# main--/rust-lz-fear

Hardware: AMD Instinct MI355X
Metric: GiB/s compress + decompress, 4 MiB independent blocks, 1/2/4/8 MI355X (higher is better)
Workload: dtype u8

## Files before the change

rust-lz-fear_amd/csrc/lz4_decompress_batch_phase.inc:

```
            LZF_STAGE_NEEDS(jv, DecodeJob); LZF_STAGE_NEEDS(rg.kRing, uint32_t); LZF_STAGE_NEEDS(sb.kCB, uint32_t); LZF_STAGE_NEEDS(lane, uint32_t);
            LZF_STAGE_NEEDS(o, uint32_t); LZF_STAGE_NEEDS(safe, uint32_t); LZF_STAGE_NEEDS(status, int); LZF_STAGE_NEEDS(cstart, uint32_t); LZF_STAGE_NEEDS(Tc, uint32_t);
            static_assert(kSpanMax + kNearHist == rg.kRing, "a batch's span and the intact history share the ring");
#if defined(LZF_FED_DECODE)
            LZF_STAGE_NEEDS(expect, uint32_t); LZF_STAGE_NEEDS(fed_carry, uint32_t); LZF_STAGE_NEEDS(bail, bool); LZF_STAGE_NEEDS(toks[0], uint16_t);
#elif !defined(LZF_TOKEN_AT)
#error "lz4_decompress_batch_phase.inc: define LZF_TOKEN_AT(i) (or LZF_FED_DECODE) around the include"
#endif
            uint32_t tidx = 0;
            if (LZF_DBG_SKIP & 1) { tidx = Tc; o += Tc; }
#if defined(LZF_FED_DECODE)
            if (LZF_DBG_SKIP & 1) expect = jv.len;
#endif
            while (tidx < Tc && status == LZF_OK) {
#if defined(LZF_FED_DECODE)
                if (lzf_fedw_carry(Tc, tidx, cstart + kRound, jv.len, fed_carry)) break;
#endif
                PHASE(0);
#if defined(LZF_DBG_ROUNDS) && defined(LZF_DBG_ROUNDS_HERE)
                ++dbg_batches;
#endif
#if defined(LZF_FED_DECODE) && defined(LZF_DBG_FED_COUNT)
                ++dbg_fed[0];
#endif
                const uint32_t ob0 = o;
                const uint32_t nb_try = Tc - tidx < kWave ? Tc - tidx : kWave;
#if defined(LZF_FED_DECODE)
                const unsigned long long act0 = lanes_below(nb_try);
#else
                const bool act0 = lane < nb_try;
#endif
                uint32_t L = 0, M = 0, src = 0;
                bool has = false;
#if defined(LZF_FED_DECODE)
                uint32_t next;
                const uint32_t pos = toks[tidx + lane_sel(act0, lane, 0u)];
                const uint32_t tp = cstart + pos;
                uint32_t w;
                asm volatile("ds_read_b32 %0, %1\n\ts_waitcnt lgkmcnt(0)" : "=v"(w) : "v"(sb.lds + pos) : "memory");
                const uint32_t l0 = (w >> 4) & 15u, b1 = (w >> 8) & 255u, m0 = w & 15u;
                const bool lx = l0 == 15u;
                const uint32_t lext = lx ? b1 : 0u;
                L = l0 + lext;
                src = tp + (lx ? 2u : 1u);
                const uint32_t q = src + L;
                has = q + 2u <= jv.len;
                const bool mx = has && m0 == 15u;
                uint32_t rq = q - cstart;
                const bool fit4 = rq + 4u <= sb.kCB;
                const uint32_t ow = lds_ld32(sb.lds + (fit4 ? rq : 0u));
                uint32_t off = ow & 0xFFFFu;
                const uint32_t mext = mx ? (fit4 ? (ow >> 16) & 255u : 255u) : 0u;
                M = has ? m0 + 4u + mext : 0u;
                uint32_t need = has ? q + (mx ? 3u : 2u) : q;
                next = has ? need : jv.len;
                const bool general = (lext > mext ? lext : mext) == 255u;
                {
                    if (general) {
                        uint32_t p = tp + 1u, b = 0;
                        bool bad = false;
                        L = l0; M = 0; has = false; next = jv.len;
                        if (lx) {
                            do { if (p >= jv.len) { bad = true; break; } b = sb.rdb(p); ++p; L += b; if (L > kMaxPosB) L = kMaxPosB; } while (b == 255u);
                        }
                        src = p;
                        if (!bad && jv.len - p < L) bad = true;
                        p += L;
                        if (!bad && jv.len - p >= 2u) {
                            has = true; p += 2u; M = m0;
                            if (m0 == 15u) {
                                do { if (p >= jv.len) { bad = true; break; } b = sb.rdb(p); ++p; M += b; if (M > kMaxPosB) M = kMaxPosB; } while (b == 255u);
                            }
                            M += 4u; next = p;
                        }
                        need = bad ? 0xFFFFFFFFu : 0u;
                        rq = sb.kCB;
                    }
                }
                if ((__builtin_amdgcn_uicmp(need, jv.len, 34 ) | __builtin_amdgcn_uicmp(tp, wave_prev(next, expect), 33 )) & act0) { bail = true; break; }
#else
#ifdef LZF_TOKEN_WORD
                bool decode = act0;
                if (act0) {
                    const uint32_t tw = LZF_TOKEN_WORD(tidx + lane);
                    const uint32_t lc = (tw >> 16) & 255u, mc = tw >> 24;
                    if (lc != 255u && mc != 255u) {
                        decode = false;
                        L = lc; src = cstart + (tw & 0xFFFFu) + (lc >= 15u ? 2u : 1u);
                        if (mc != 254u) { has = true; M = mc + 4u; }
                    }
                }
                if (decode) {
#else
                if (act0) {
#endif
                    const uint32_t tp = cstart + LZF_TOKEN_AT(tidx + lane);
                    const uint32_t w = sb.rd4(tp);
                    const uint32_t tok = w & 255u;
                    uint32_t q = tp + 1u;
                    L = tok >> 4;
                    if (L == 15u) {
                        uint32_t b = (w >> 8) & 255u; ++q;
                        L += b;
                        while (b == 255u) { b = sb.rdb(q); ++q; L += b; if (L > kMaxPosB) L = kMaxPosB; }
                    }
                    src = q; q += L;
                    if (jv.len - q >= 2u) {
                        has = true; q += 2u;
                        M = tok & 15u;
                        if (M == 15u) { for (;;) { const uint32_t b = sb.rdb(q); ++q; M += b; if (M > kMaxPosB) M = kMaxPosB; if (b != 255u) break; } }
                        M += 4u;
                    }
                }
#endif
                uint32_t tot = L + M; if (tot > kTotClamp || tot < L) tot = kTotClamp;
#if defined(LZF_FED_DECODE)
                const uint32_t tot0 = lane_sel(act0, tot, 0u);
                const uint32_t incl = wave_scan_add(tot0);
                const uint32_t lo = ob0 + (incl - tot0);
                const uint32_t mo = lo + L;
                const uint32_t nb = first_lane_min(__builtin_amdgcn_uicmp(incl, kSpanMax, 34 ), nb_try);
#else
                const uint32_t incl = wave_scan_add(act0 ? tot : 0u);
                const uint32_t lo = ob0 + (incl - (act0 ? tot : 0u));
                const uint32_t mo = lo + L;
                const uint32_t c = first_lane(__ballot(act0 && incl > kSpanMax));
                const uint32_t nb = c < nb_try ? c : nb_try;
#endif

                if (nb == 0u) {
#if defined(LZF_FED_DECODE)
                    expect = __builtin_amdgcn_readlane(next, 0);
#endif
                    const uint32_t s_L = __builtin_amdgcn_readlane(L, 0);
                    const uint32_t s_M = __builtin_amdgcn_readlane(M, 0);
                    const uint32_t s_src = __builtin_amdgcn_readlane(src, 0);
                    const bool s_has = __builtin_amdgcn_readlane((uint32_t)has, 0) != 0u;
                    if (jv.cap - o < s_L) { status = LZF_OUT_CAPACITY; break; }
                    if (s_has && (uint64_t)o + s_L + s_M > jv.limit) { status = LZF_MEMORY_LIMIT_EXCEEDED; break; }
                    const uint32_t o_before = o;
                    wave_copy(jv.out + o, jv.in + s_src, s_L, lane);
                    o += s_L;
                    if (s_has) {
                        const uint32_t offset = (uint32_t)jv.in[s_src + s_L] | ((uint32_t)jv.in[s_src + s_L + 1u] << 8);
                        uint32_t mlen = s_M;
                        if (offset == 0u) { status = LZF_ZERO_DEDUP_OFFSET; break; }
                        bool done = false;
                        if (offset > o) {
                            const uint32_t need = offset - o;
                            if (need > jv.plen) { status = LZF_INVALID_DEDUP_OFFSET; break; }
                            const uint32_t nn = need < mlen ? need : mlen;
                            if (jv.cap - o < nn) { status = LZF_OUT_CAPACITY; break; }
                            wave_copy(jv.out + o, jv.prefix + (jv.plen - need), nn, lane);
                            o += nn; mlen -= nn;
                            done = mlen == 0u;
                        }
                        if (!done) {
                            if (jv.cap - o < mlen) { status = LZF_OUT_CAPACITY; break; }
                            const uint32_t src0 = o - offset;
                            const uint32_t span = mlen < offset ? mlen : offset;
                            if (src0 + span > safe) { wave_store_fence(); safe = o; }
                            cgu8* hist = jv.out + src0;
                            gu8* dst = jv.out + o;
                            if (mlen <= offset) {
                                wave_copy(dst, hist, mlen, lane);
                            } else if (offset == 1u) {
                                const uint32_t b = hist[0];
                                const uint32_t b4 = b * 0x01010101u;
                                const u32x4 v = {b4, b4, b4, b4};
                                const uint32_t bulk = mlen & ~15u;
                                for (uint32_t i = lane * 16u; i < bulk; i += kWave * 16u) st16(dst + i, v);
                                if (lane < mlen - bulk) dst[bulk + lane] = (uint8_t)b;
                            } else {
                                uint32_t r = lane % offset;
                                const uint32_t adv = kWave % offset;
                                for (uint32_t i = lane; i < mlen; i += kWave) {
                                    dst[i] = hist[r];
                                    r += adv; if (r >= offset) r -= offset;
                                }
                            }
                            o += mlen;
                        }
                    }
                    wave_store_fence(); safe = o;
                    rg.fill((o - o_before > rg.kRing) ? o - rg.kRing : o_before, o);
                    tidx += 1u;
                    continue;
                }

#if defined(LZF_FED_DECODE)
                expect = __builtin_amdgcn_readlane(next, nb - 1u);
                const unsigned long long act_m = lanes_below(nb);
                L = lane_sel(act_m, L, 0u); M = lane_sel(act_m, M, 0u);
                has = M != 0u;
                const unsigned long long has_m = __builtin_amdgcn_uicmp(M, 0u, 33 );
                const bool act = lane < nb;
                if (__builtin_amdgcn_uicmp(rq, sb.kCB - 4u, 34 ) & has_m) {
                    asm volatile("");
                    if (has && rq > sb.kCB - 4u) {
                        if (!sb.kStage) off = ld2(jv.in + src + L);
                        else if (src + L - cstart + 2u <= sb.kCB) off = lds_ld16(sb.lds + (src + L - cstart));
                        else off = sb.rdb(src + L) | (sb.rdb(src + L + 1u) << 8);
                    }
                }
#else
                const bool act = lane < nb;
                has = has && act;
                if (!act) { L = 0; M = 0; }
                uint32_t off = 0;
                if (has) {
                    if (!sb.kStage) off = ld2(jv.in + src + L);
                    else if (src + L - cstart + 2u <= sb.kCB) off = lds_ld16(sb.lds + (src + L - cstart));
                    else off = sb.rdb(src + L) | (sb.rdb(src + L + 1u) << 8);
                }
#endif
#if defined(LZF_FED_DECODE)
                static_assert(kSpanMax < kTotClamp && (uint64_t)kMaxPosB * 2u < (1ull << 32), "the bounds argument above");
                const uint32_t lim32 = jv.limit > 0xFFFFFFFFull ? 0xFFFFFFFFu : (uint32_t)jv.limit;
                const uint32_t fit = jv.cap < lim32 ? jv.cap : lim32;
                const uint32_t E = ob0 + __builtin_amdgcn_readlane(incl, nb - 1u);
                const unsigned long long flagged = (__builtin_amdgcn_uicmp(off - 1u, mo + jv.plen, 35 ) & has_m) | __builtin_amdgcn_uicmp(E, fit, 34 );
                if (flagged) {
#endif
                int code = LZF_OK;
                if (act) {
                    if (lo > jv.cap || jv.cap - lo < L) code = LZF_OUT_CAPACITY;
                    else if (has && (uint64_t)mo + M > jv.limit) code = LZF_MEMORY_LIMIT_EXCEEDED;
                    else if (has && off == 0u) code = LZF_ZERO_DEDUP_OFFSET;
                    else if (has && off > mo && off - mo > jv.plen) code = LZF_INVALID_DEDUP_OFFSET;
                    else if (has && jv.cap - mo < M) code = LZF_OUT_CAPACITY;
                }
                const uint32_t e = first_lane(__ballot(code != LZF_OK));
                if (e < 64u) { status = __builtin_amdgcn_readlane(code, e); break; }
#if defined(LZF_FED_DECODE)
                }
#endif
                PHASE(1);

                const uint32_t near_lo = ob0 > kNearHist ? ob0 - kNearHist : 0u;
                const uint32_t span = M < off ? M : off;
                const bool from_prefix = has && off > mo;
                const uint32_t s0 = mo - off;
                const bool is_near = has && !from_prefix && s0 >= near_lo;
                const bool is_far = has && !from_prefix && s0 + span <= near_lo;
                const bool is_slow = has && !is_near && !is_far;
                const uint32_t mi = RIDX(mo);
                const bool mwrap = mi + M > rg.kRing;
                {
                    uint32_t need = 0;
                    if (is_far) need = s0 + M;
                    if (is_slow && !from_prefix) need = near_lo;
                    if (is_slow && from_prefix && M > off - mo) need = near_lo;
                    if (need > ob0) need = ob0;
                    if (__ballot(need > safe)) { wave_store_fence(); safe = ob0; }
                }
                const bool far_own = !(LZF_DBG_SKIP & 4) && is_far && M <= kFarShort && !mwrap;
                uint64_t fv0 = 0, fv1 = 0, fv2 = 0, fv3 = 0;
#ifndef LZF_FAR_LATE
                if (far_own) {
                    cgu8* g = jv.out + s0;
                    if (M >= 8u) {
                        fv0 = ld8(g); fv3 = ld8(g + M - 8u);
                        if (M > 16u) { fv1 = ld8(g + 8u); fv2 = ld8(g + M - 16u); }
                    } else {
                        fv0 = ld4(g); fv3 = ld4(g + M - 4u);
                    }
                }
#endif
                if (!(LZF_DBG_SKIP & 8) && __ballot(L > 0u)) {
                    const uint32_t n1 = L < kShort ? L : kShort;
                    const uint32_t ri = RIDX(lo);
                    if (n1 > 0u) {
                        if (ri + n1 > rg.kRing) {
                            for (uint32_t t = 0; t < n1; ++t) rg.ring[RIDX(lo + t)] = (uint8_t)sb.rdb(src + t);
                        } else if (sb.kStage && src - cstart + n1 <= sb.kCB) {
                            put_small_lds(rg.lds + ri, sb.lds + (src - cstart), n1);
                        } else {
                            put_small_glb(rg.lds + ri, jv.in + src, n1);
                        }
                    }
                    for (unsigned long long m = __ballot(L > kShort); m; m &= m - 1ull) {
                        const uint32_t j = (uint32_t)__builtin_ctzll(m);
                        const uint32_t jl = __builtin_amdgcn_readlane(L, j);
                        const uint32_t js = __builtin_amdgcn_readlane(src, j);
                        const uint32_t jo = __builtin_amdgcn_readlane(lo, j);
                        for (uint32_t i = kShort + lane; i < jl; i += 4u * kWave) {
                            const uint32_t i1 = i + kWave, i2 = i + 2u * kWave, i3 = i + 3u * kWave;
                            const uint8_t b0 = jv.in[js + i];
                            const uint8_t b1 = i1 < jl ? jv.in[js + i1] : (uint8_t)0;
                            const uint8_t b2 = i2 < jl ? jv.in[js + i2] : (uint8_t)0;
                            const uint8_t b3 = i3 < jl ? jv.in[js + i3] : (uint8_t)0;
                            rg.ring[RIDX(jo + i)] = b0;
                            if (i1 < jl) rg.ring[RIDX(jo + i1)] = b1;
                            if (i2 < jl) rg.ring[RIDX(jo + i2)] = b2;
                            if (i3 < jl) rg.ring[RIDX(jo + i3)] = b3;
                        }
                    }
                }
                PHASE(2);

#ifdef LZF_FAR_LATE
                if (far_own) {
                    cgu8* g = jv.out + s0;
                    if (M >= 8u) {
                        fv0 = ld8(g); fv3 = ld8(g + M - 8u);
                        if (M > 16u) { fv1 = ld8(g + 8u); fv2 = ld8(g + M - 16u); }
                    } else {
                        fv0 = ld4(g); fv3 = ld4(g + M - 4u);
                    }
                }
#endif
                if (far_own) {
                    const uint32_t dsta = rg.lds + mi;
                    if (M >= 8u) {
                        lds_st64(dsta, fv0);
                        if (M > 16u) { lds_st64(dsta + 8u, fv1); lds_st64(dsta + M - 16u, fv2); }
                        lds_st64(dsta + M - 8u, fv3);
                    } else {
                        lds_st32(dsta, (uint32_t)fv0); lds_st32(dsta + M - 4u, (uint32_t)fv3);
                    }
                }
                if (!(LZF_DBG_SKIP & 4) && __ballot(is_far && !far_own)) {
                    if (is_far && M <= kShort && mwrap) { for (uint32_t t = 0; t < M; ++t) rg.ring[RIDX(mo + t)] = jv.out[s0 + t]; }
                    if (is_far && M > kFarShort && M <= kShort && !mwrap) put_small_glb(rg.lds + mi, jv.out + s0, M);
                    for (unsigned long long m = __ballot(is_far && M > kShort); m; m &= m - 1ull) {
                        const uint32_t j = (uint32_t)__builtin_ctzll(m);
                        const uint32_t jm = __builtin_amdgcn_readlane(M, j);
                        const uint32_t js = __builtin_amdgcn_readlane(s0, j);
                        const uint32_t jo = __builtin_amdgcn_readlane(mo, j);
                        for (uint32_t i = lane; i < jm; i += 4u * kWave) {
                            const uint32_t i1 = i + kWave, i2 = i + 2u * kWave, i3 = i + 3u * kWave;
                            const uint8_t b0 = jv.out[js + i];
                            const uint8_t b1 = i1 < jm ? jv.out[js + i1] : (uint8_t)0;
                            const uint8_t b2 = i2 < jm ? jv.out[js + i2] : (uint8_t)0;
                            const uint8_t b3 = i3 < jm ? jv.out[js + i3] : (uint8_t)0;
                            rg.ring[RIDX(jo + i)] = b0;
                            if (i1 < jm) rg.ring[RIDX(jo + i1)] = b1;
                            if (i2 < jm) rg.ring[RIDX(jo + i2)] = b2;
                            if (i3 < jm) rg.ring[RIDX(jo + i3)] = b3;
                        }
                    }
                }
                PHASE(3);
                unsigned long long unresolved = __ballot(is_near || is_slow);
                const unsigned long long slow_mask = __ballot(is_slow);
                {
                    const uint32_t si = RIDX(s0);
                    const bool solo_ok = is_near && M <= off && M <= kShort && !mwrap && !(si + M > rg.kRing);
                    const unsigned long long solo_mask = __ballot(solo_ok);
                    uint32_t src_end = solo_ok ? s0 + span : 0xFFFFFFFFu;
                    if (LZF_DBG_SKIP & 2) unresolved = 0;
                    while (unresolved) {
#if defined(LZF_DBG_ROUNDS) && defined(LZF_DBG_ROUNDS_HERE)
                        ++dbg_rounds;
#endif
#if defined(LZF_FED_DECODE) && defined(LZF_DBG_FED_COUNT)
                        ++dbg_fed[3];
#endif
                        const uint32_t f = (uint32_t)__builtin_ctzll(unresolved);
                        const unsigned long long bit = 1ull << f;
                        if (solo_mask & bit) {
                            const uint32_t H = __builtin_amdgcn_readlane(mo, f);
                            const bool mine = src_end <= H;
                            if (mine) { put_match_lds(rg.lds + mi, rg.lds + si, M); src_end = 0xFFFFFFFFu; }
#if defined(LZF_DBG_ROUNDS) && defined(LZF_DBG_ROUNDS_HERE) && LZF_DBG_ROUNDS >= 3
                            { const uint32_t nl = (uint32_t)__builtin_popcountll(__ballot(mine));
                              dbg_lane_stat += LZF_DBG_ROUNDS == 3 ? nl : LZF_DBG_ROUNDS == 4 ? 1u : LZF_DBG_ROUNDS == 5 ? (nl == 1u) : LZF_DBG_ROUNDS == 6 ? (nl >= 2u && nl <= 4u)
                                             : LZF_DBG_ROUNDS == 7 ? (nl >= 5u && nl <= 16u) : (nl >= 17u); }
#endif
                            unresolved &= ~__ballot(mine);
                            continue;
                        }
                        unresolved &= ~bit;
                        if (slow_mask & bit) {
                            if (lane == f) {
                                for (uint32_t t = 0; t < M; ++t) {
                                    uint8_t v;
                                    if (off > mo + t) v = jv.prefix[jv.plen - (off - mo) + t];
                                    else {
                                        const uint32_t s = mo + t - off;
                                        v = s < near_lo ? jv.out[s] : rg.ring[RIDX(s)];
                                    }
                                    rg.ring[RIDX(mo + t)] = v;
                                }
                            }
                            continue;
                        }
                        const uint32_t jm = __builtin_amdgcn_readlane(M, f);
                        const uint32_t js = __builtin_amdgcn_readlane(s0, f);
                        const uint32_t jo = __builtin_amdgcn_readlane(mo, f);
                        const uint32_t joff = __builtin_amdgcn_readlane(off, f);
                        if (jm <= joff) {
                            for (uint32_t i = lane; i < jm; i += 4u * kWave) {
                                const uint32_t i1 = i + kWave, i2 = i + 2u * kWave, i3 = i + 3u * kWave;
                                const uint8_t b0 = rg.ring[RIDX(js + i)];
                                const uint8_t b1 = i1 < jm ? rg.ring[RIDX(js + i1)] : (uint8_t)0;
                                const uint8_t b2 = i2 < jm ? rg.ring[RIDX(js + i2)] : (uint8_t)0;
                                const uint8_t b3 = i3 < jm ? rg.ring[RIDX(js + i3)] : (uint8_t)0;
                                rg.ring[RIDX(jo + i)] = b0;
                                if (i1 < jm) rg.ring[RIDX(jo + i1)] = b1;
                                if (i2 < jm) rg.ring[RIDX(jo + i2)] = b2;
                                if (i3 < jm) rg.ring[RIDX(jo + i3)] = b3;
                            }
#if defined(LZF_FED_DECODE)
                        } else if ((LZF_DBG_SKIP & 64) && joff <= 8u && ((0x116u >> joff) & 1u)) {
#endif
                        } else {
#if defined(LZF_FED_DECODE) && !defined(LZF_FED_NO_PERIODIC)
                            uint32_t rr = lane & (joff - 1u), adv = kWave & (joff - 1u);
                            if ((joff & (joff - 1u)) != 0u) {
                                asm volatile("");
                                rr = lane % joff; adv = kWave % joff;
                            }
#if defined(LZF_DBG_FED_COUNT)
                            dbg_fed[4] += (joff & (joff - 1u)) == 0u ? 1u : 0u;
#endif
#else
                            uint32_t rr = lane % joff;
                            const uint32_t adv = kWave % joff;
#endif
                            for (uint32_t i = lane; i < jm; i += kWave) {
                                rg.ring[RIDX(jo + i)] = rg.ring[RIDX(js + rr)];
                                rr += adv; if (rr >= joff) rr -= joff;
                            }
                        }
                    }
                }
                PHASE(4);
                o = ob0 + __builtin_amdgcn_readlane(incl, (nb - 1u) & 63u);
                if (!(LZF_DBG_SKIP & 16)) rg.flush(ob0, o);
                tidx += nb;
                PHASE(5);
            }
```

rust-lz-fear_amd/csrc/lz4_decompress_fed.hip:

```cpp
#include "lzf_device.h"
#include "kernels.h"
#include "lzf_copy_helpers.h"
#include "lzf_phase_timers.h"
#include "lzf_fed_window.h"
#include "lzf_dispatch.h"

namespace lzf {

__device__ __forceinline__ uint32_t xcc_id() {
    uint32_t v; asm volatile("s_getreg_b32 %0, hwreg(HW_REG_XCC_ID)" : "=s"(v)); return v & 15u;
}

template <int RING, int W, int TOKCAP>
__global__ LZF_FED_BOUNDS void lzf_decompress_fed_kernel(fed_args a) {
    constexpr uint32_t kSpanMax = RING / 3;
    constexpr uint32_t kNearHist = RING - kSpanMax;
    constexpr uint32_t kRound = 32u * (uint32_t)W;
    constexpr uint32_t kCB = kRound + 128u;
    static_assert(W >= 1 && W <= 64 && kRound == (uint32_t)kFedwRound, "a window is one bit-map word per lane (whose owner is worked out per word: lzf_fed_window.h)");
    static_assert(TOKCAP >= (int)(kRound / 3u + 1u), "a round's tokens (at least three bytes each) fit the list");
    static_assert(kCB % 16 == 0, "the round is staged in 16-byte pieces");
    __shared__ __attribute__((aligned(16))) uint8_t ring[RING];
    __shared__ __attribute__((aligned(16))) uint8_t cbuf[kCB];
    __shared__ __attribute__((aligned(16))) uint16_t toks[TOKCAP];
    static_assert(RING != 4096 || W != 32 || TOKCAP != 352 || lzf_dispatch::lds_alloc(sizeof ring + sizeof cbuf + sizeof toks) == lzf_dispatch::kFedLdsAlloc, "lzf_dispatch.h: the residency the census falls back on");

    const uint32_t lane = threadIdx.x;
    if (a.census) {
        if (lane == 0u) {
            __hip_atomic_fetch_or(&a.census[2], 1u << (xcc_id() & 31u), __ATOMIC_RELAXED, __HIP_MEMORY_SCOPE_AGENT);
            __hip_atomic_fetch_add(&a.census[0], 1u, __ATOMIC_RELAXED, __HIP_MEMORY_SCOPE_AGENT);
            const unsigned long long t0 = wall_clock64();
            while (wall_clock64() - t0 < 30000ull) __builtin_amdgcn_s_sleep(16);
            const uint32_t seen = __hip_atomic_load(&a.census[0], __ATOMIC_RELAXED, __HIP_MEMORY_SCOPE_AGENT);
            __hip_atomic_fetch_min(&a.census[1], seen, __ATOMIC_RELAXED, __HIP_MEMORY_SCOPE_AGENT);
        }
        return;
    }
    const uint32_t n = a.n_jobs, pieces = a.pieces;
    const uint32_t xcc = xcc_id() & 31u;
    if (pieces > 1u && !((a.xcc_mask >> xcc) & 1u)) return;
    const uint32_t ng = pieces > 1u ? (uint32_t)__popc(a.xcc_mask) : 1u, g = pieces > 1u ? (uint32_t)__popc(a.xcc_mask & ((1u << xcc) - 1u)) : 0u;
    const uint32_t n_g = lzf_fedw_group_jobs(n, g, ng);
#ifdef LZF_ANALYSIS
    const uint32_t n_tickets = n_g * (a.stop_piece && a.stop_piece < pieces ? a.stop_piece : pieces);
#else
    const uint32_t n_tickets = n_g * pieces;
#endif
    for (;;) {
    uint32_t tk = 0;
    if (lane == 0u) tk = __hip_atomic_fetch_add(a.ticket + g * kFedTicketStride, 1u, __ATOMIC_RELAXED, __HIP_MEMORY_SCOPE_AGENT);
    tk = __builtin_amdgcn_readfirstlane(tk);
    if (tk >= n_tickets) break;
    const uint32_t piece = lzf_fedw_ticket_piece(tk, n_g), k = lzf_fedw_ticket_rank(tk, piece, n_g, g, ng);
    const uint32_t jid = a.perm ? a.perm[k] : k;
    const seg_job sj = a.st[jid];
    if (!sj.eligible || sj.failed || sj.done) continue;
    LZF_GLOBAL fed_state* const fs = (LZF_GLOBAL fed_state*)a.state + jid;
    const lzf_decompress_job job = a.jobs[jid];
    const long long t_start = clock64();
#ifdef LZF_DBG_TIMELINE
    const unsigned long long t_wall0 = wall_clock64();
#endif

    int status = LZF_OK;
    bool bailed = false, parked = false;
    uint32_t o = 0;
    PhaseTimers ph;
#ifdef LZF_DBG_FED_COUNT
    uint32_t dbg_fed[5] = {0u, 0u, 0u, 0u, 0u};
#endif
    if (LZF_DECODE_JOB_OUT_OF_CONTRACT(job)) continue;
    {
        const DecodeJob jv = LZF_DECODE_JOB_VIEW(job);
        const OutRing<RING> rg{ring, jv.out, jv.rb, lane, lds_addr(ring)};
        const uint32_t cbuf_a = lds_addr(cbuf);
        const LZF_GLOBAL uint32_t* const fed_bits = (const LZF_GLOBAL uint32_t*)a.bits + (size_t)jid * a.maxch * kSegChunkWords;
        uint32_t expect = 0;
        uint32_t cstart = 0;
        o = (uint32_t)job.out_existing_len;
        const uint32_t piece_end = lzf_fedw_piece_end(jv.len, pieces, piece);
        if (piece > 0u) {
            uint32_t f = 0;
            for (uint32_t spin = 0; spin < (1u << 22); ++spin) {
                f = __hip_atomic_load(&fs->flag, __ATOMIC_RELAXED, __HIP_MEMORY_SCOPE_AGENT);
                if (f >= piece) break;
                __builtin_amdgcn_s_sleep(32);
            }
            f = __builtin_amdgcn_readfirstlane(f);
            if (f != piece) continue;
            __builtin_amdgcn_fence(__ATOMIC_ACQUIRE, "agent");
            expect = fs->expect; o = fs->o;
        }
        uint32_t safe = o;
        if (o > 0) rg.fill(o > (uint32_t)RING ? o - RING : 0u, o);
        ph.start();
#if defined(LZF_FED_FIXED_ROUNDS)
        constexpr int kFixed = 1;
        const uint32_t fed_carry = 0u;
#elif defined(LZF_ANALYSIS)
        constexpr int kFixed = 0;
        const uint32_t fed_carry = a.carry < kWave ? a.carry : kWave - 1u;
#else
        constexpr int kFixed = 0;
        constexpr uint32_t fed_carry = kFedwCarry;
#endif
        bool fed_walk = false;
        while (expect < jv.len && status == LZF_OK) {
            if (expect >= piece_end) { parked = true; break; }
            const uint32_t expect_in = expect;
            cstart = lzf_fedw_start(expect, kFixed);
            __syncthreads();
#ifdef LZF_DBG_FED_COUNT
            ++dbg_fed[fed_walk ? 2 : 1];
#endif
#include "lz4_decompress_feed_phase.inc"
            if (Tc) {
#define LZF_FED_DECODE
#ifdef LZF_FED_FAR_LATE
#define LZF_FAR_LATE
#endif
#include "lz4_decompress_batch_phase.inc"
#undef LZF_FAR_LATE
#undef LZF_FED_DECODE
            }
            if (bail) {
                if (fed_walk) { bailed = true; break; }
                fed_walk = true; continue;
            }
            fed_walk = false;
            if (expect == expect_in && status == LZF_OK) { bailed = true; break; }
        }
        if (parked && status == LZF_OK && !bailed) {
            if (lane == 0u) { fs->expect = expect; fs->o = o; }
            __builtin_amdgcn_fence(__ATOMIC_RELEASE, "workgroup");
            asm volatile("s_waitcnt vmcnt(0)" ::: "memory");
            if (lane == 0u) __hip_atomic_store(&fs->flag, piece + 1u, __ATOMIC_RELAXED, __HIP_MEMORY_SCOPE_AGENT);
            continue;
        }
    }
    if (pieces > 1u && lane == 0u) __hip_atomic_store(&fs->flag, kFedEnded, __ATOMIC_RELAXED, __HIP_MEMORY_SCOPE_AGENT);
    if (bailed || status != LZF_OK) continue;
    if (lane == 0) {
        a.results[jid].out_len = o;
        a.results[jid].status = LZF_OK;
#ifdef LZF_DBG_FED_COUNT
        a.results[jid].reserved = dbg_fed[LZF_DBG_FED_COUNT];
#elif defined(LZF_DBG_PHASE_SEL)
        ph.report(a.results[jid]);
#elif defined(LZF_DBG_TIMELINE)
        a.results[jid].reserved = (uint32_t)(((t_wall0 >> 8) & 0xFFFFull) << 16) | (uint32_t)((wall_clock64() >> 8) & 0xFFFFull);
#else
        a.results[jid].reserved = (uint32_t)((clock64() - t_start) >> 10);
#endif
        a.st[jid].done = 1u;
    }
    }
}

__global__ __launch_bounds__(256) void lzf_fed_reset_kernel(fed_args a) {
    const uint32_t k = blockIdx.x * blockDim.x + threadIdx.x;
    if (k < 32u) a.ticket[k * kFedTicketStride] = 0u;
    if (k < a.n_jobs) a.state[k].flag = 0u;
}

#define LZF_INSTF(NAME, RG, W_, T) template __global__ void lzf_decompress_fed_kernel<RG, W_, T>(fed_args);
LZF_FED_VARIANTS(LZF_INSTF)
#undef LZF_INSTF

}
```

rust-lz-fear_amd/csrc/lzf_out_ring.h:

```cpp
#ifndef LZF_OUT_RING_H
#define LZF_OUT_RING_H

#include <stdint.h>
#if defined(__HIPCC__) || defined(__CUDACC__)
#define LZF_RING_HD __host__ __device__
#else
#define LZF_RING_HD
#endif
struct lzf_ring_parts { uint32_t head, vec, tail; };

LZF_RING_HD constexpr lzf_ring_parts lzf_ring_split(uint32_t a, uint32_t b, uint32_t rb) {
    uint32_t nh = (16u - ((a + rb) & 15u)) & 15u;
    if (nh > b - a) nh = b - a;
    a += nh;
    const uint32_t nv = (b - a) >> 4;
    a += nv << 4;
    return lzf_ring_parts{nh, nv, b - a};
}

#if defined(__HIPCC__)
#include "lzf_device.h"

namespace lzf {
namespace {

#define RIDX(x) (((x) + rg.rb) & (rg.kRing - 1u))
template <int RING>
struct OutRing {
    static_assert(RING >= 16 && (RING & (RING - 1)) == 0, "ring index = address mod RING");
    static constexpr uint32_t kRing = RING;
    uint8_t* ring;
    gu8* out;
    uint32_t rb;
    uint32_t lane;
    uint32_t lds;
    __device__ __forceinline__ uint32_t idx(uint32_t x) const { const OutRing& rg = *this; return RIDX(x); }
    __device__ __forceinline__ uint8_t& at(uint32_t x) const { return ring[idx(x)]; }
    template <bool FLUSH>
    __device__ __forceinline__ void move(uint32_t a, uint32_t b) const {
        const lzf_ring_parts s = lzf_ring_split(a, b, rb);
        if (lane < s.head) { if (FLUSH) out[a + lane] = at(a + lane); else at(a + lane) = out[a + lane]; }
        a += s.head;
        for (uint32_t c = lane; c < s.vec; c += kWave) {
            LZF_GLOBAL u32x4* const g = reinterpret_cast<LZF_GLOBAL u32x4*>(out + a + 16u * c);
            u32x4* const r = reinterpret_cast<u32x4*>(&at(a + 16u * c));
            if (FLUSH) *g = *r; else *r = *g;
        }
        a += s.vec << 4;
        if (lane < s.tail) { if (FLUSH) out[a + lane] = at(a + lane); else at(a + lane) = out[a + lane]; }
    }
    __device__ __forceinline__ void fill(uint32_t a, uint32_t b) const { move<false>(a, b); }
    __device__ __forceinline__ void flush(uint32_t a, uint32_t b) const { move<true>(a, b); }
};

}
}
#endif
#endif
```

Measured before the change: 545.3.

## Defer ring flush of each batch into the next batch's match phase

Result: faster. 552.2 (median of 6 runs) (+1.3%).

```diff
diff --git a/rust-lz-fear_amd/csrc/lz4_decompress_batch_phase.inc b/rust-lz-fear_amd/csrc/lz4_decompress_batch_phase.inc
--- a/rust-lz-fear_amd/csrc/lz4_decompress_batch_phase.inc
+++ b/rust-lz-fear_amd/csrc/lz4_decompress_batch_phase.inc
@@ -2,14 +2,15 @@
             LZF_STAGE_NEEDS(o, uint32_t); LZF_STAGE_NEEDS(safe, uint32_t); LZF_STAGE_NEEDS(status, int); LZF_STAGE_NEEDS(cstart, uint32_t); LZF_STAGE_NEEDS(Tc, uint32_t);
             static_assert(kSpanMax + kNearHist == rg.kRing, "a batch's span and the intact history share the ring");
 #if defined(LZF_FED_DECODE)
-            LZF_STAGE_NEEDS(expect, uint32_t); LZF_STAGE_NEEDS(fed_carry, uint32_t); LZF_STAGE_NEEDS(bail, bool); LZF_STAGE_NEEDS(toks[0], uint16_t);
+            LZF_STAGE_NEEDS(expect, uint32_t); LZF_STAGE_NEEDS(fed_carry, uint32_t); LZF_STAGE_NEEDS(bail, bool); LZF_STAGE_NEEDS(toks[0], uint16_t); LZF_STAGE_NEEDS(pend, uint32_t);
+            static_assert(kSpanMax + 16u <= kNearHist, "the batch before and the ragged end before it lie inside the history this batch keeps intact, above every far source");
 #elif !defined(LZF_TOKEN_AT)
 #error "lz4_decompress_batch_phase.inc: define LZF_TOKEN_AT(i) (or LZF_FED_DECODE) around the include"
 #endif
             uint32_t tidx = 0;
             if (LZF_DBG_SKIP & 1) { tidx = Tc; o += Tc; }
 #if defined(LZF_FED_DECODE)
-            if (LZF_DBG_SKIP & 1) expect = jv.len;
+            if (LZF_DBG_SKIP & 1) { expect = jv.len; pend = o; }
 #endif
             while (tidx < Tc && status == LZF_OK) {
 #if defined(LZF_FED_DECODE)
@@ -130,6 +131,8 @@
                 if (nb == 0u) {
 #if defined(LZF_FED_DECODE)
                     expect = __builtin_amdgcn_readlane(next, 0);
+                    if (!(LZF_DBG_SKIP & 16)) rg.flush(pend, o);
+                    pend = 0xFFFFFFFFu;
 #endif
                     const uint32_t s_L = __builtin_amdgcn_readlane(L, 0);
                     const uint32_t s_M = __builtin_amdgcn_readlane(M, 0);
@@ -183,6 +186,9 @@
                     }
                     wave_store_fence(); safe = o;
                     rg.fill((o - o_before > rg.kRing) ? o - rg.kRing : o_before, o);
+#if defined(LZF_FED_DECODE)
+                    pend = o;
+#endif
                     tidx += 1u;
                     continue;
                 }
@@ -251,7 +257,16 @@
                     if (is_slow && !from_prefix) need = near_lo;
                     if (is_slow && from_prefix && M > off - mo) need = near_lo;
                     if (need > ob0) need = ob0;
+#if defined(LZF_FED_DECODE)
+                    if (__ballot(need > safe)) {
+#if defined(LZF_DBG_FED_COUNT)
+                        ++dbg_fed[5];
+#endif
+                        wave_store_fence(); safe = pend;
+                    }
+#else
                     if (__ballot(need > safe)) { wave_store_fence(); safe = ob0; }
+#endif
                 }
                 const bool far_own = !(LZF_DBG_SKIP & 4) && is_far && M <= kFarShort && !mwrap;
                 uint64_t fv0 = 0, fv1 = 0, fv2 = 0, fv3 = 0;
@@ -341,6 +356,12 @@
                     }
                 }
                 PHASE(3);
+#if defined(LZF_FED_DECODE)
+                __builtin_amdgcn_s_waitcnt(0x0F70);
+                if (LZF_DBG_SKIP & 128) { rg.flush_dry(pend, ob0); pend = ob0; }
+                else if (LZF_DBG_SKIP & 16) pend = ob0;
+                else pend = rg.flush_lines(pend, ob0);
+#endif
                 unsigned long long unresolved = __ballot(is_near || is_slow);
                 const unsigned long long slow_mask = __ballot(is_slow);
                 {
@@ -427,7 +448,10 @@
                 }
                 PHASE(4);
                 o = ob0 + __builtin_amdgcn_readlane(incl, (nb - 1u) & 63u);
+#if defined(LZF_FED_DECODE)
+#else
                 if (!(LZF_DBG_SKIP & 16)) rg.flush(ob0, o);
+#endif
                 tidx += nb;
                 PHASE(5);
             }
diff --git a/rust-lz-fear_amd/csrc/lz4_decompress_fed.hip b/rust-lz-fear_amd/csrc/lz4_decompress_fed.hip
--- a/rust-lz-fear_amd/csrc/lz4_decompress_fed.hip
+++ b/rust-lz-fear_amd/csrc/lz4_decompress_fed.hip
@@ -68,7 +68,7 @@
     uint32_t o = 0;
     PhaseTimers ph;
 #ifdef LZF_DBG_FED_COUNT
-    uint32_t dbg_fed[5] = {0u, 0u, 0u, 0u, 0u};
+    uint32_t dbg_fed[6] = {0u, 0u, 0u, 0u, 0u, 0u};
 #endif
     if (LZF_DECODE_JOB_OUT_OF_CONTRACT(job)) continue;
     {
@@ -93,6 +93,7 @@
             expect = fs->expect; o = fs->o;
         }
         uint32_t safe = o;
+        uint32_t pend = o;
         if (o > 0) rg.fill(o > (uint32_t)RING ? o - RING : 0u, o);
         ph.start();
 #if defined(LZF_FED_FIXED_ROUNDS)
@@ -131,6 +132,7 @@
             fed_walk = false;
             if (expect == expect_in && status == LZF_OK) { bailed = true; break; }
         }
+        if (pend < o && !(LZF_DBG_SKIP & 16)) rg.flush(pend, o);
         if (parked && status == LZF_OK && !bailed) {
             if (lane == 0u) { fs->expect = expect; fs->o = o; }
             __builtin_amdgcn_fence(__ATOMIC_RELEASE, "workgroup");
diff --git a/rust-lz-fear_amd/csrc/lzf_out_ring.h b/rust-lz-fear_amd/csrc/lzf_out_ring.h
--- a/rust-lz-fear_amd/csrc/lzf_out_ring.h
+++ b/rust-lz-fear_amd/csrc/lzf_out_ring.h
@@ -51,6 +51,29 @@
     }
     __device__ __forceinline__ void fill(uint32_t a, uint32_t b) const { move<false>(a, b); }
     __device__ __forceinline__ void flush(uint32_t a, uint32_t b) const { move<true>(a, b); }
+    __device__ __forceinline__ uint32_t flush_lines(uint32_t a, uint32_t b) const {
+        const uint32_t nh = (0u - (a + rb)) & 15u;
+        if (nh != 0u) {
+            if (b - a < nh) return a;
+            if (lane < nh) out[a + lane] = at(a + lane);
+            a += nh;
+        }
+        const uint32_t nv = (b - a) >> 4;
+        for (uint32_t c = lane; c < nv; c += kWave)
+            *reinterpret_cast<LZF_GLOBAL u32x4*>(out + a + 16u * c) = *reinterpret_cast<u32x4*>(&at(a + 16u * c));
+        return a + (nv << 4);
+    }
+    __device__ __forceinline__ void flush_dry(uint32_t a, uint32_t b) const {
+        const lzf_ring_parts s = lzf_ring_split(a, b, rb);
+        if (lane < s.head) { const uint32_t v = at(a + lane); asm volatile("" :: "v"(v), "v"(out + a + lane)); }
+        a += s.head;
+        for (uint32_t c = lane; c < s.vec; c += kWave) {
+            const u32x4 v = *reinterpret_cast<u32x4*>(&at(a + 16u * c));
+            asm volatile("" :: "v"(v), "v"(out + a + 16u * c));
+        }
+        a += s.vec << 4;
+        if (lane < s.tail) { const uint32_t v = at(a + lane); asm volatile("" :: "v"(v), "v"(out + a + lane)); }
+    }
 };
 
 }
```
